# richardbaihe/a3t

Measured on AMD Instinct MI355X. Metric: mel-frames/sec (train), higher is better.
Workload: dtype bf16; 1 GPU; VCTK A3T masked-mel train step: 6+6 Conformer blocks d=384 H=2 ff=1536(k3), B=32/GPU, T_mel=1000, T_phn=120, postnet 5x256x5, fwd+bwd+clip+Adam, dropout 0.2/0.2/0.2 + postnet 0.5 (recipe); global_batch=32, parallelism=dp1, params=100799808

## Files before the change

a3t_amd/_lib.py:

```python
import ctypes
import os
from ctypes import POINTER, c_char_p, c_float, c_int, c_int32, c_int64, c_void_p

import torch

HERE = os.path.dirname(os.path.abspath(__file__))
LIB_PATH = os.environ.get("A3T_LIB_PATH") or os.path.join(HERE, "lib", "liba3t_hip.so")

F32, BF16 = 0, 1
ACT_NONE, ACT_RELU, ACT_TANH, ACT_SWISH = 0, 1, 2, 3
ACC_STORE, ACC_ADD, ACC_ATOMIC, ACC_SOLE = 0, 1, 2, 3


class GemmDesc(ctypes.Structure):
    _fields_ = [
        ("A", c_void_p), ("B", c_void_p), ("C", c_void_p), ("bias", c_void_p), ("R", c_void_p), ("S", c_void_p),
        ("M", c_int32), ("N", c_int32), ("K", c_int32),
        ("a_rs", c_int64), ("a_cs", c_int64),
        ("b_rs", c_int64), ("b_cs", c_int64), ("b_ts", c_int64),
        ("c_rs", c_int64),
        ("batch", c_int32), ("batch_inner", c_int32),
        ("a_bs0", c_int64), ("a_bs1", c_int64), ("b_bs0", c_int64), ("b_bs1", c_int64),
        ("c_bs0", c_int64), ("c_bs1", c_int64),
        ("taps", c_int32), ("pad", c_int32), ("dil", c_int32), ("Tseq", c_int32), ("kshift", c_int32),
        ("alpha", c_float),
        ("act", c_int32), ("accumulate", c_int32), ("splitk", c_int32),
        ("a_dtype", c_int32), ("b_dtype", c_int32), ("c_dtype", c_int32), ("compute", c_int32),
        ("s_dtype", c_int32), ("colsum_slots", c_int32),
        ("colsum", c_void_p), ("colsum_bs1", c_int64), ("colsum_scale", c_float), ("drop_key", ctypes.c_uint32),
        ("drop_p", c_float), ("colsum_ss", c_int32),
        ("keep_out", c_void_p), ("keep_in", c_void_p),
        ("a_signmask", c_int32), ("keep_layout", c_int32),
        ("A2", c_void_p), ("B2", c_void_p), ("b2_cs", c_int64), ("b2_bs0", c_int64), ("b2_bs1", c_int64), ("colsum2", c_void_p),
        ("a2_rs", c_int64), ("a_unaligned", c_int32),
    ]


_P = c_void_p
_SIGS = {
    "a3t_gemm": [POINTER(GemmDesc), _P],
    "a3t_gemm_plan": [POINTER(GemmDesc), c_char_p, c_int],
    "a3t_layernorm_fwd": [_P, _P, _P, _P, c_int, _P, _P, c_int, c_int, c_float, _P],
    "a3t_layernorm_bwd": [_P, c_int, _P, _P, _P, _P, _P, _P, _P, _P, _P, _P, c_float, c_int, c_int, c_float,
                          ctypes.c_uint32, _P],
    "a3t_col_reduce": [_P, c_int, _P, _P, _P, _P, c_int, c_int, c_int64, c_int, _P],
    "a3t_f64_to_f32_add": [_P, _P, c_int, c_float, _P],
    "a3t_bn_act_fwd": [_P, _P, _P, _P, _P, _P, _P, _P, _P, c_int, c_int, c_int, c_float, c_float, c_int, c_int, _P],
    "a3t_bn_act_bwd_a": [_P, c_int, _P, _P, _P, _P, _P, _P, c_int, c_int, c_int, _P],
    "a3t_bn_act_bwd_b": [_P, c_int, _P, _P, _P, _P, _P, _P, _P, _P, _P, c_int, c_int, c_int, c_int, _P],
    "a3t_glu_dwconv_fwd": [_P, c_int, _P, _P, _P, c_int, _P, c_int, c_int, c_int, c_int, _P],
    "a3t_glu_dwconv_bwd": [_P, _P, c_int, _P, c_int, _P, _P, c_int, _P, _P, _P, c_int, c_int, c_int, c_int, _P],
    "a3t_add_pos_bias": [_P, _P, _P, _P, _P, c_int, c_int, c_int, _P],
    "a3t_add_pos_bias_bwd": [_P, _P, _P, c_int, c_int, c_int, _P],
    "a3t_relpos_softmax_fwd": [_P, _P, c_int, _P, _P, c_int, c_int, c_int, c_int, c_int64, c_int64, c_int64, c_float, _P,
                               c_float, ctypes.c_uint32, _P],
    "a3t_relpos_softmax_bwd": [_P, c_int, _P, c_int, _P, _P, c_int, c_int, c_int, c_int, c_int64, c_int64, c_int64, c_float, _P,
                               c_float, c_int64, c_int64, ctypes.c_uint32, _P, _P],
    "a3t_attn_fwd_train": [_P, _P, _P, _P, _P, _P, _P, _P, _P, _P, _P, c_int, c_int, c_int, c_int, c_int64, c_int64, c_int64,
                           c_int64, c_float, c_float, ctypes.c_uint32, _P, _P, _P],
    "a3t_attn_scale_rows": [_P, _P, _P, c_int, c_int, c_int, c_int, _P],
    "a3t_attn_bwd_ds": [_P, _P, _P, _P, _P, _P, _P, c_int, c_int, c_int, c_int, c_int64, c_int64, c_int64, c_int64, c_float,
                        c_float, ctypes.c_uint32, c_int, c_int64, _P],
    "a3t_attn_fwd": [_P, _P, _P, _P, _P, _P, _P, _P, c_int, c_int, c_int, c_int, c_int64, c_int64, c_int64, c_int64,
                     c_float, c_float, ctypes.c_uint32, _P, _P, _P],
    "a3t_pwg_block": [_P, _P, _P, _P, _P, _P, _P, _P, c_int, c_int, c_int, _P],
    "a3t_mask_fill": [_P, _P, _P, _P, c_int, c_int, c_int, _P],
    "a3t_embed_finish_fwd": [_P, _P, _P, _P, _P, _P, _P, c_int, c_int, c_int, c_int, c_float, c_float, ctypes.c_uint32,
                             _P, _P],
    "a3t_embed_finish_bwd": [_P, _P, _P, _P, _P, _P, _P, _P, c_int, c_int, c_int, c_int, c_int, c_int, c_float, c_float,
                             ctypes.c_uint32, _P],
    "a3t_scale": [_P, _P, c_int64, c_float, _P],
    "a3t_axpy": [_P, _P, c_int64, c_float, _P],
    "a3t_attn_bias_fold": [_P, c_int32, c_int32, _P, _P, _P, _P],
    "a3t_scale_dev": [_P, _P, c_int64, _P, _P],
    "a3t_slice_rows": [_P, _P, c_int, c_int, c_int, c_int, c_int, c_int, _P],
    "a3t_cast_bf16": [_P, _P, c_int64, _P],
    "a3t_cast_bf16_conv_t": [_P, _P, _P, _P, c_int, c_int, c_int, c_int, _P],
    "a3t_split_bf16": [_P, _P, _P, c_int64, _P],
    "a3t_reflect_pad": [_P, _P, c_int, c_int, c_int, c_int, _P],
    "a3t_stft_amp": [_P, _P, c_int64, c_int, c_int, _P],
    "a3t_logmel_finish": [_P, _P, c_int, c_int, c_int, _P],
    "a3t_mlm_loss": [_P, _P, _P, _P, _P, _P, _P, _P, c_int, c_int, c_int, c_float, _P],
    "a3t_mlm_loss_scratch_floats": [c_int],
    "a3t_sumsq": [_P, c_int64, _P, _P],
# ... 62 lines not shown
```

a3t_amd/csrc/convmod_attn.hip:

```cpp
#include <hip/hip_runtime.h>
#include <stdint.h>
#include "../../include/a3t_hip.h"
#include "dtype_io.h"

#define WAVE 64
__device__ __forceinline__ float sigm(float v) { return 1.f / (1.f + __expf(-v)); }
__device__ __forceinline__ float bf2f_(unsigned int h) { return __uint_as_float(h << 16); }
__device__ __forceinline__ float wsum(float v) {
#pragma unroll
    for (int o = 32; o > 0; o >>= 1) v += __shfl_xor(v, o, WAVE);
    return v;
}
__device__ __forceinline__ float wmax(float v) {
#pragma unroll
    for (int o = 32; o > 0; o >>= 1) v = fmaxf(v, __shfl_xor(v, o, WAVE));
    return v;
}

#define DW_TT 64
#define DW_KMAX 31

template <int KT>
__global__ __launch_bounds__(256) void glu_dwconv_fwd_kernel(const void* __restrict__ g, int g_dt,
                                                             const float* __restrict__ wdw,
// ... 38 lines not shown
#pragma unroll
            for (int j = 0; j < KT + 3; ++j) v[j] = win[r0 + j][tx];
#pragma unroll
            for (int tt = 0; tt < 4; ++tt) {
                float acc = bias;
#pragma unroll
                for (int k = 0; k < KT; ++k) acc += w[k] * v[tt + k];
                int t = t0 + r0 + tt;
                if (t < Tseq) z[(mbase + t) * (int64_t)C + c] = acc;
            }
        }
        return;
    }
    for (int r = ty; r < DW_TT; r += 4) {
        int t = t0 + r;
        if (t >= Tseq) break;
        float acc = bias;
#pragma unroll
        for (int k = 0; k < KT; ++k)
            if (k < K) acc += w[k] * win[r + k][tx];
        z[(mbase + t) * (int64_t)C + c] = acc;
    }
}

int a3t_glu_dwconv_fwd_vec(const void* g, const float* wdw, const float* bdw, void* glu, float* z, int M, int C, int K,
                           int Tseq, hipStream_t stream);
int a3t_glu_dwconv_bwd_vec(const float* dz, const void* g, const void* glu, const float* wdw, void* dg, float* dwdw,
                           float* dbdw, float* dg_colsum, int M, int C, int K, int Tseq, hipStream_t stream);
static inline bool dw_al16(const void* p) { return ((uintptr_t)p & 15) == 0; }

extern "C" int a3t_glu_dwconv_fwd(const void* g, int g_dtype, const float* wdw, const float* bdw, void* glu,
                                  int glu_dtype, float* z, int M, int C, int K, int Tseq, void* stream) {
    if (K > DW_KMAX || (K & 1) == 0 || Tseq <= 0 || M % Tseq) return A3T_EINVAL;
    if (g_dtype == A3T_BF16 && glu_dtype == A3T_BF16 && C % 64 == 0 && dw_al16(g) && dw_al16(glu) && dw_al16(z))
        return a3t_glu_dwconv_fwd_vec(g, wdw, bdw, glu, z, M, C, K, Tseq, (hipStream_t)stream);
    int B = M / Tseq, tiles_t = (Tseq + DW_TT - 1) / DW_TT;
    dim3 grid((C + 63) / 64, B * tiles_t);
    if (K <= 7)
        hipLaunchKernelGGL(glu_dwconv_fwd_kernel<7>, grid, dim3(256), 0, (hipStream_t)stream, g, g_dtype, wdw, bdw, glu,
                           glu_dtype, z, C, K, Tseq, tiles_t);
    else if (K <= 15)
        hipLaunchKernelGGL(glu_dwconv_fwd_kernel<15>, grid, dim3(256), 0, (hipStream_t)stream, g, g_dtype, wdw, bdw, glu,
                           glu_dtype, z, C, K, Tseq, tiles_t);
    else
        hipLaunchKernelGGL(glu_dwconv_fwd_kernel<DW_KMAX>, grid, dim3(256), 0, (hipStream_t)stream, g, g_dtype, wdw, bdw,
                           glu, glu_dtype, z, C, K, Tseq, tiles_t);
    return (int)hipGetLastError();
}

template <int KT>
__global__ __launch_bounds__(256, 3) void glu_dwconv_bwd_kernel(const float* __restrict__ dz, const void* __restrict__ g,
                                                             int g_dt, const void* __restrict__ glu, int glu_dt,
                                                             const float* __restrict__ wdw, void* __restrict__ dg,
                                                             int dg_dt, float* dwdw, float* dbdw, float* dgsum, int C,
                                                             int K, int Tseq, int tiles_t, int tiles_per_block,
                                                             int chunks) {
    __shared__ float wdz[DW_TT + DW_KMAX - 1][64];
    __shared__ float wgl[DW_TT + DW_KMAX - 1][64];
    __shared__ float red[4][64];
    const int tx = threadIdx.x & 63, ty = threadIdx.x >> 6;
    const int c = blockIdx.x * 64 + tx;
    const int b = blockIdx.y / chunks, tile0 = (blockIdx.y % chunks) * tiles_per_block;
    const int pad = (K - 1) / 2;
    const int64_t mbase = (int64_t)b * Tseq;
    const int rows = DW_TT + K - 1;
    float w[KT], dw[KT];
#pragma unroll
    for (int k = 0; k < KT; ++k) {
// ... 661 lines not shown
```

a3t_amd/csrc/dwconv_vec.hip:

```cpp
#include <hip/hip_runtime.h>
#include <stdint.h>
#include "../../include/a3t_hip.h"
#include "dtype_io.h"

#define DW_TT 64
#define DW_KMAX 31
typedef unsigned short u16;

__device__ __forceinline__ float dv_sigm(float v) { return 1.f / (1.f + __expf(-v)); }
__device__ __forceinline__ float dv_bf(unsigned int h) { return __uint_as_float(h << 16); }
__device__ __forceinline__ void dv_unpack8(const uint4& u, float* f) {
    f[0] = dv_bf(u.x & 0xffff), f[1] = dv_bf(u.x >> 16), f[2] = dv_bf(u.y & 0xffff), f[3] = dv_bf(u.y >> 16);
    f[4] = dv_bf(u.z & 0xffff), f[5] = dv_bf(u.z >> 16), f[6] = dv_bf(u.w & 0xffff), f[7] = dv_bf(u.w >> 16);
}
__device__ __forceinline__ uint4 dv_pack8(const float* f) {
    uint4 u;
    u.x = io_pack2(f[0], f[1]), u.y = io_pack2(f[2], f[3]);
    u.z = io_pack2(f[4], f[5]), u.w = io_pack2(f[6], f[7]);
    return u;
}

template <int KT>
__global__ __launch_bounds__(256) void glu_dwconv_fwd_vec_kernel(const u16* __restrict__ g, const float* __restrict__ wdw,
                                                                 const float* __restrict__ bdw, u16* __restrict__ glu,
                                                                 float* __restrict__ z, int C, int K, int Tseq,
                                                                 int tiles_t) {
    __shared__ __attribute__((aligned(16))) float win[DW_TT + DW_KMAX - 1][64];
    __shared__ __attribute__((aligned(16))) float zt[DW_TT][64];
    const int tid = threadIdx.x, tx = tid & 63, ty = tid >> 6;
    const int cblk = blockIdx.x * 64, c = cblk + tx;
    const int b = blockIdx.y / tiles_t, t0 = (blockIdx.y % tiles_t) * DW_TT;
    const int pad = (K - 1) / 2;
    const int64_t mbase = (int64_t)b * Tseq;
    const int rows = DW_TT + K - 1;
    {
        const int rr = tid >> 3, c8 = (tid & 7) * 8;
        uint4 av[3], bv[3];
#pragma unroll
        for (int ps = 0; ps < 3; ++ps) {
            const int r = ps * 32 + rr, t = t0 - pad + r;
            const bool ok = (r < rows) && (t >= 0) && (t < Tseq);
            const u16* src = g + (ok ? (mbase + t) * (int64_t)(2 * C) + cblk + c8 : 0);
            av[ps] = *(const uint4*)src;
            bv[ps] = *(const uint4*)(src + (ok ? C : 0));
        }
#pragma unroll
        for (int ps = 0; ps < 3; ++ps) {
            const int r = ps * 32 + rr, t = t0 - pad + r;
            const bool ok = (r < rows) && (t >= 0) && (t < Tseq);
            if (r < rows) {
                float a[8], bb[8], v[8];
                dv_unpack8(av[ps], a);
                dv_unpack8(bv[ps], bb);
#pragma unroll
                for (int e = 0; e < 8; ++e) v[e] = ok ? a[e] * dv_sigm(bb[e]) : 0.f;
                *(float4*)&win[r][c8] = make_float4(v[0], v[1], v[2], v[3]);
                *(float4*)&win[r][c8 + 4] = make_float4(v[4], v[5], v[6], v[7]);
                if (ok && r >= pad && r < pad + DW_TT) *(uint4*)(glu + (mbase + t) * (int64_t)C + cblk + c8) = dv_pack8(v);
            }
        }
    }
    __syncthreads();
    float w[KT];
#pragma unroll
    for (int k = 0; k < KT; ++k) w[k] = (k < K) ? wdw[(int64_t)c * K + k] : 0.f;
    const float bias = bdw[c];
    if (K == KT) {
        for (int r0 = ty * 4; r0 < DW_TT; r0 += 16) {
            float v[KT + 3];
#pragma unroll
            for (int j = 0; j < KT + 3; ++j) v[j] = win[r0 + j][tx];
#pragma unroll
            for (int tt = 0; tt < 4; ++tt) {
                float acc = bias;
#pragma unroll
                for (int k = 0; k < KT; ++k) acc = __builtin_fmaf(w[k], v[tt + k], acc);
                zt[r0 + tt][tx] = acc;
            }
        }
    } else {
        for (int r = ty; r < DW_TT; r += 4) {
            float acc = bias;
#pragma unroll
            for (int k = 0; k < KT; ++k)
                if (k < K) acc += w[k] * win[r + k][tx];
            zt[r][tx] = acc;
        }
    }
    __syncthreads();
    {
        const int rr = tid >> 4, c4 = (tid & 15) * 4;
// ... 161 lines not shown
                if (t < Tseq) {
                    u16* dst = dg + (mbase + t) * (int64_t)(2 * C) + cblk + c8;
                    *(uint4*)dst = *(const uint4*)&gt[0][r][c8];
                    *(uint4*)(dst + C) = *(const uint4*)&gt[1][r][c8];
                }
            }
        }
    }
    __syncthreads();
    float* part = &wdz[0][0];
    for (int i = tid; i < 64 * K; i += 256) part[i] = 0.f;
    __syncthreads();
#pragma unroll
    for (int k = 0; k < KT; ++k)
        if (k < K) atomicAdd(&part[tx * K + k], dw[k]);
    __syncthreads();
    for (int i = tid; i < 64 * K; i += 256) atomicAdd(&dwdw[(int64_t)cblk * K + i], part[i]);
    __syncthreads();
    red[ty][tx] = db;
    __syncthreads();
    if (ty == 0) atomicAdd(&dbdw[c], red[0][tx] + red[1][tx] + red[2][tx] + red[3][tx]);
    if (dgsum) {
        __syncthreads();
        red[ty][tx] = sga;
        __syncthreads();
        if (ty == 0) atomicAdd(&dgsum[c], red[0][tx] + red[1][tx] + red[2][tx] + red[3][tx]);
        __syncthreads();
        red[ty][tx] = sgb;
        __syncthreads();
        if (ty == 0) atomicAdd(&dgsum[C + c], red[0][tx] + red[1][tx] + red[2][tx] + red[3][tx]);
    }
}

int a3t_glu_dwconv_bwd_vec(const float* dz, const void* g, const void* glu, const float* wdw, void* dg, float* dwdw,
                           float* dbdw, float* dg_colsum, int M, int C, int K, int Tseq, hipStream_t stream) {
    const int B = M / Tseq, tiles_t = (Tseq + DW_TT - 1) / DW_TT;
    const int cb = C / 64;
    int chunks = 1;
    while (cb * B * chunks < 640 && chunks < tiles_t) ++chunks;
    const int tpb = (tiles_t + chunks - 1) / chunks;
    chunks = (tiles_t + tpb - 1) / tpb;
    dim3 grid(cb, B * chunks);
#define DWB(KT)                                                                                                       \
    hipLaunchKernelGGL(glu_dwconv_bwd_vec_kernel<KT>, grid, dim3(256), 0, stream, dz, (const u16*)g, (const u16*)glu, \
                       wdw, (u16*)dg, dwdw, dbdw, dg_colsum, C, K, Tseq, tiles_t, tpb, chunks)
    if (K <= 7)
        DWB(7);
    else if (K <= 15)
        DWB(15);
    else
        DWB(DW_KMAX);
#undef DWB
    return (int)hipGetLastError();
}
```

a3t_amd/csrc/norm_reduce.hip:

```cpp
#include <hip/hip_runtime.h>
#include <stdlib.h>
#include <stdint.h>
#include "../../include/a3t_hip.h"
#include "dtype_io.h"

#define WAVE 64

__device__ __forceinline__ float wave_sum(float v) {
#pragma unroll
    for (int o = 32; o > 0; o >>= 1) v += __shfl_xor(v, o, WAVE);
    return v;
}

#define LN_MAXV 24

template <int V>
__global__ __launch_bounds__(256) void ln_fwd_kernel(const float* __restrict__ x, const float* __restrict__ g,
                                                     const float* __restrict__ b, void* __restrict__ y, int y_dt,
                                                     float* __restrict__ mean, float* __restrict__ rstd, int M,
                                                     int D, float eps) {
    const int lane = threadIdx.x & 63, wv = threadIdx.x >> 6;
    const int row = blockIdx.x * 4 + wv;
    if (row >= M) return;
    const float* xr = x + (int64_t)row * D;
    float v[V];
    float s = 0.f;
#pragma unroll
    for (int i = 0; i < V; ++i) {
        int c = lane + i * 64;
        v[i] = (c < D) ? xr[c] : 0.f;
        s += v[i];
    }
    const float mu = wave_sum(s) / (float)D;
    float q = 0.f;
#pragma unroll
    for (int i = 0; i < V; ++i) {
        int c = lane + i * 64;
// ... 382 lines not shown
}

__global__ void f64_to_f32_add_kernel(const double* src, float* dst, int n, float scale) {
    int i = blockIdx.x * blockDim.x + threadIdx.x;
    if (i < n) dst[i] += (float)(src[i] * (double)scale);
}
extern "C" int a3t_f64_to_f32_add(const double* src, float* dst, int n, float scale, void* stream) {
    hipLaunchKernelGGL(f64_to_f32_add_kernel, dim3((n + 255) / 256), dim3(256), 0, (hipStream_t)stream, src, dst, n,
                       scale);
    return (int)hipGetLastError();
}

__global__ void bn_finalize_kernel(const double* stats, float* running_mean, float* running_var, float* mean_out,
                                   float* rstd_out, int M, int C, float eps, float momentum, int training) {
    int c = blockIdx.x * blockDim.x + threadIdx.x;
    if (c >= C) return;
    if (training) {
        double mu = stats[c] / (double)M;
        double var = stats[C + c] / (double)M - mu * mu;
        if (var < 0.0) var = 0.0;
        mean_out[c] = (float)mu;
        rstd_out[c] = (float)(1.0 / sqrt(var + (double)eps));
        if (momentum > 0.f && running_mean) {
            double unb = (M > 1) ? var * (double)M / (double)(M - 1) : var;
            running_mean[c] = (1.f - momentum) * running_mean[c] + momentum * (float)mu;
            running_var[c] = (1.f - momentum) * running_var[c] + momentum * (float)unb;
        }
    } else {
        mean_out[c] = running_mean[c];
        rstd_out[c] = 1.0f / sqrtf(running_var[c] + eps);
    }
}

__device__ __forceinline__ float sigmoidf_(float v) { return 1.f / (1.f + __expf(-v)); }

__global__ __launch_bounds__(256) void bn_act_fwd_kernel(const float* __restrict__ z, const float* __restrict__ mean,
                                                         const float* __restrict__ rstd,
                                                         const float* __restrict__ gamma,
                                                         const float* __restrict__ beta, void* __restrict__ y,
                                                         int y_dt, int64_t n, int C, int act, int vec) {
    if (vec) {
        const int64_t n4 = n >> 2;
        for (int64_t q = (int64_t)blockIdx.x * blockDim.x + threadIdx.x; q < n4; q += (int64_t)gridDim.x * blockDim.x) {
            const int64_t i = q << 2;
            const int c = (int)(i % C);
            const float4 zv = *(const float4*)(z + i);
            const float4 mu = *(const float4*)(mean + c), rs = *(const float4*)(rstd + c);
            const float4 g = *(const float4*)(gamma + c), b = *(const float4*)(beta + c);
            float o[4] = {(zv.x - mu.x) * rs.x * g.x + b.x, (zv.y - mu.y) * rs.y * g.y + b.y,
                          (zv.z - mu.z) * rs.z * g.z + b.z, (zv.w - mu.w) * rs.w * g.w + b.w};
#pragma unroll
            for (int e = 0; e < 4; ++e) {
                if (act == A3T_ACT_SWISH)
                    o[e] = o[e] * sigmoidf_(o[e]);
                else if (act == A3T_ACT_TANH)
                    o[e] = tanhf(o[e]);
            }
            if (y_dt == A3T_BF16) {
                uint2 h;
                h.x = io_pack2(o[0], o[1]);
                h.y = io_pack2(o[2], o[3]);
                *(uint2*)((unsigned short*)y + i) = h;
            } else {
                *(float4*)((float*)y + i) = make_float4(o[0], o[1], o[2], o[3]);
            }
        }
        return;
    }
    for (int64_t i = (int64_t)blockIdx.x * blockDim.x + threadIdx.x; i < n; i += (int64_t)gridDim.x * blockDim.x) {
        int c = (int)(i % C);
        float bn = (z[i] - mean[c]) * rstd[c] * gamma[c] + beta[c];
        float o = bn;
        if (act == A3T_ACT_SWISH)
            o = bn * sigmoidf_(bn);
        else if (act == A3T_ACT_TANH)
            o = tanhf(bn);
        stx(y, y_dt, i, o);
    }
}

extern "C" int a3t_bn_act_fwd(const float* z, const double* stats, const float* gamma, const float* beta,
                              float* running_mean, float* running_var, float* mean_out, float* rstd_out, void* y,
                              int y_dtype, int M, int C, float eps, float momentum, int training, int act,
                              void* stream) {
    hipStream_t s = (hipStream_t)stream;
    hipLaunchKernelGGL(bn_finalize_kernel, dim3((C + 255) / 256), dim3(256), 0, s, stats, running_mean, running_var,
                       mean_out, rstd_out, M, C, eps, momentum, training);
    int64_t n = (int64_t)M * C;
    const int vec = (C % 4 == 0 && ((uintptr_t)z % 16 == 0) && ((uintptr_t)y % 16 == 0) && ((uintptr_t)mean_out % 16 == 0) &&
                     ((uintptr_t)rstd_out % 16 == 0) && ((uintptr_t)gamma % 16 == 0) && ((uintptr_t)beta % 16 == 0)) ? 1 : 0;
    int blocks = (int)(((vec ? n / 4 : n) + 255) / 256);
    if (blocks > 4096) blocks = 4096;
    hipLaunchKernelGGL(bn_act_fwd_kernel, dim3(blocks), dim3(256), 0, s, z, mean_out, rstd_out, gamma, beta, y, y_dtype, n,
                       C, act, vec);
    return (int)hipGetLastError();
}

__device__ __forceinline__ float bn_dact(float d, float bn, int act) {
    if (act == A3T_ACT_SWISH) {
        const float sg = sigmoidf_(bn);
        return d * sg * (1.f + bn * (1.f - sg));
    }
    if (act == A3T_ACT_TANH) {
        const float t = tanhf(bn);
        return d * (1.f - t * t);
    }
    return d;
}

__global__ __launch_bounds__(256) void bn_act_bwd_a_kernel(const void* __restrict__ dy, int dy_dt, const float* __restrict__ z,
                                                           const float* __restrict__ mean,
                                                           const float* __restrict__ rstd,
                                                           const float* __restrict__ gamma,
                                                           const float* __restrict__ beta,
                                                           double* sums, int M, int C, int act, int rows_per_block) {
    __shared__ double red[2][4][64];
    const int tx = threadIdx.x & 63, ty = threadIdx.x >> 6;
    const int c = blockIdx.x * 64 + tx;
    const int r0 = blockIdx.y * rows_per_block, r1 = min(M, r0 + rows_per_block);
    double a0 = 0.0, a1 = 0.0;
    if (c < C) {
        const float mu = mean[c], rs = rstd[c], g = gamma[c], b = beta[c];
        float f0 = 0.f, f1 = 0.f;
        int cnt = 0;
        for (int r = r0 + ty; r < r1; r += 4) {
            int64_t i = (int64_t)r * C + c;
            float zh = (z[i] - mu) * rs;
            float d = bn_dact(ldx(dy, dy_dt, i), zh * g + b, act);
            f0 += d;
            f1 += d * zh;
            if (++cnt == 32) {
                a0 += f0, a1 += f1, f0 = f1 = 0.f, cnt = 0;
            }
        }
        a0 += f0, a1 += f1;
    }
    red[0][ty][tx] = a0;
    red[1][ty][tx] = a1;
    __syncthreads();
    if (ty == 0 && c < C) {
// ... 118 lines not shown
```

a3t_amd/engine.py:

```python
import math
import os
import zlib
from typing import Dict

import torch

from . import ops
from ._lib import ACC_ADD, ACC_ATOMIC, ACC_STORE, ACT_NONE, ACT_RELU, ACT_SWISH, ACT_TANH, BF16, F32
from .config import A3TConfig
from .params import ParamStore


def legacy_pe_table(c: A3TConfig) -> torch.Tensor:
    d = c.adim
    position = torch.arange(c.max_len - 1, -1, -1.0, dtype=torch.float32).unsqueeze(1)
    div = torch.exp(torch.arange(0, d, 2, dtype=torch.float32) * -(math.log(10000.0) / d))
    pe = torch.zeros(c.max_len, d)
    pe[:, 0::2] = torch.sin(position * div)
    pe[:, 1::2] = torch.cos(position * div)
    return pe


_STREAMS = {}

# ... 653 lines not shown
            self._bias_grad(dqu, gr[pre + ".u"])
            self._bias_grad(dqv, gr[pre + ".v"])
            self._bias_grad(dqkv, gbq)
        self._lin_wgrad(dqkv, y, gr[pre + ".wqkv"])
        dy = self._act("tmp.dy", (M, d))
        self._lin_dgrad(dqkv, pre + ".wqkv", dy)
        self._pre_ln(ga, g, g16)
        self._ln_bwd(tag + ".ln", dy, pre + ".ln", g, g, g16, nb, nxt)
        self._sub_end()
        return g

    def _bn_fwd(self, tag, z, pre, bufpre, act, out):
        p, b = self.store.p, self.store.buf
        M, C = z.shape
        stats = self._arena_slot("fwd64", tag + ".stats", 2 * C)
        if self.training:
            ops.col_reduce(z, stats[:C], stats[C:], mode=1)
        mean = self.ws.get(tag + ".bnmean", (C,))
        rstd = self.ws.get(tag + ".bnrstd", (C,))
        ops.bn_act_fwd(z, stats, p[pre + ".g"], p[pre + ".b"], b[bufpre + ".rm"], b[bufpre + ".rv"], mean, rstd, out,
                       1e-5, self.bn_momentum if self.training else 0.0, self.training, act)
        if self.training:
            self.store.nbt[bufpre] = self.store.nbt.get(bufpre, 0) + 1
        self.sv[tag + ".bn"] = (z, mean, rstd)

    def _bn_bwd(self, tag, dy, pre, act, dz):
        p, gr = self.store.p, self.store.g
        z, mean, rstd = self.sv[tag + ".bn"]
        M, C = z.shape
        sums = self._arena_slot("bwd64", tag + ".bnsums", 2 * C)
        ops.bn_act_bwd(dy, z, mean, rstd, p[pre + ".g"], p[pre + ".b"], sums, dz, gr[pre + ".g"], gr[pre + ".b"],
                       self.training, act, zero=False)

    def _conv_fwd(self, tag, pre, x, T):
        p, c = self.store.p, self.c
        M, d = x.shape
        cmp = self.cmp
        y = self._ln_fwd(tag + ".ln", x, pre + ".ln")
        g2 = self._act(tag + ".g", (M, 2 * d))
        ops.linear_fwd(y, self.W(pre + ".pw1"), g2, bias=p[pre + ".pb1"], compute=cmp)
        glu = self._act(tag + ".glu", (M, d))
        z = self.ws.get(tag + ".z", (M, d))
        ops.glu_dwconv_fwd(g2, p[pre + ".dw"], p[pre + ".db"], glu, z, T)
        s = self._act(tag + ".s", (M, d))
        self._bn_fwd(tag, z, pre + ".bn", pre + ".bn", ACT_SWISH, s)
        xo = self.ws.get(tag + ".xo", (M, d))
        ops.linear_fwd(s, self.W(pre + ".pw2"), xo, bias=p[pre + ".pb2"], R=x, compute=cmp,
                       drop=self._drop(c.dropout_rate, tag + ".o"))
        self.sv[tag] = (y, g2, glu, s)
        return xo

    def _conv_bwd(self, tag, pre, g, T, nb=None, nxt=None):
        p, gr, c = self.store.p, self.store.g, self.c
        M, d = g.shape
        cmp = self.cmp
        y, g2, glu, s = self.sv[tag]
        self._sub_begin()
        g16 = self._g16(g)
        ga = self._gm(g, tag + ".o", c.dropout_rate, gr[pre + ".pb2"], 1.0)
        self._lin_wgrad(ga, s, gr[pre + ".pw2"])
        ds = self.ws.get("tmp.ds", (M, d))
        self._lin_dgrad(ga, pre + ".pw2", ds)
        dz = self.ws.get("tmp.dz", (M, d))
        self._bn_bwd(tag, ds, pre + ".bn", ACT_SWISH, dz)
        dg = self._act(self._t("tmp.dg"), (M, 2 * d))
        ops.glu_dwconv_bwd(dz, g2, glu, p[pre + ".dw"], dg, gr[pre + ".dw"], gr[pre + ".db"], T,
                           dgsum=gr[pre + ".pb1"])
        self._lin_wgrad(dg, y, gr[pre + ".pw1"])
        dy = self._act("tmp.dy", (M, d))
        self._lin_dgrad(dg, pre + ".pw1", dy)
        self._pre_ln(ga, g, g16)
        self._ln_bwd(tag + ".ln", dy, pre + ".ln", g, g, g16, nb, nxt)
        self._sub_end()
        return g

    def block_fwd(self, pre, x, pos, keymask, B, T):
        x = self._ffn_fwd(pre + ".ffm", pre + ".ffm", x, T)
        x = self._mha_fwd(pre + ".mha", pre + ".mha", x, pos, keymask, B, T)
        x = self._conv_fwd(pre + ".cnv", pre + ".cnv", x, T)
        x = self._ffn_fwd(pre + ".ff", pre + ".ff", x, T)
        return self._ln_fwd(pre + ".fin", x, pre + ".fin.ln", out_dtype=torch.float32)

    def block_bwd(self, pre, g, B, T):
        gr = self.store.g
        self._ln_bwd(pre + ".fin", g, pre + ".fin.ln", None, g, self._g16(g), (gr[pre + ".ff.b2"], 0.5), pre + ".ff.o")
        self._ffn_bwd(pre + ".ff", pre + ".ff", g, T, (gr[pre + ".cnv.pb2"], 1.0), pre + ".cnv.o")
        self._conv_bwd(pre + ".cnv", pre + ".cnv", g, T, (gr[pre + ".mha.bo"], 1.0), pre + ".mha.o")
        self._mha_bwd(pre + ".mha", pre + ".mha", g, B, T, (gr[pre + ".ffm.b2"], 0.5), pre + ".ffm.o")
        self._ffn_bwd(pre + ".ffm", pre + ".ffm", g, T, None)
        return g

    def forward(self, batch: Dict[str, torch.Tensor], need_grad: bool = True, gscale: float = 1.0):
        c, p, ws = self.c, self.store.p, self.ws
        speech = batch["speech"].contiguous()
        B, Tm, idim = speech.shape
        text = batch["text"].contiguous()
        Tp = text.shape[1]
        T = Tm + Tp
        d = c.adim
        if self.bf16 and (T % 8 or Tm % 8):
# ... 229 lines not shown
```

a3t_amd/ops.py:

```python
import ctypes
import os

import torch

from . import _lib as L
from ._lib import ACC_ADD, ACC_ATOMIC, ACC_SOLE, ACC_STORE, ACT_NONE, ACT_RELU, ACT_SWISH, ACT_TANH, BF16, F32

__all__ = ["gemm", "gemm_plan", "linear_fwd", "linear_bwd_data", "linear_bwd_weight", "conv_fwd", "conv_bwd_data",
           "conv_bwd_weight"]


PROFILE = None


def _stream():
    return ctypes.c_void_p(torch.cuda.current_stream().cuda_stream)


def _ptr(t):
    if t is None:
        return None
    return ctypes.c_void_p(t.data_ptr())


# ... 215 lines not shown

def layernorm_bwd(dy, x, g, mean, rstd, dres, dx, dg, db, dx16=None, dxsum=None, dxsum_scale=1.0, drop=(0.0, 0)):
    M, D = x.shape
    L.check(L.load().a3t_layernorm_bwd(_ptr(dy), _dt(dy), _ptr(x), _ptr(g), _ptr(mean), _ptr(rstd), _ptr(dres),
                                       _ptr(dx), _ptr(dx16), _ptr(dg), _ptr(db), _ptr(dxsum), dxsum_scale, M, D,
                                       drop[0], drop[1], _stream()), "ln_bwd")


def col_reduce(x, out0, out1=None, y=None, rowmask=None, mode=0, ld=None):
    M, C = x.shape
    L.check(L.load().a3t_col_reduce(_ptr(x), _dt(x), _ptr(y), _ptr(rowmask), _ptr(out0), _ptr(out1), M, C,
                                    ld if ld is not None else x.stride(0), mode, _stream()), "col_reduce")


def f64_to_f32_add(src, dst, scale=1.0):
    L.check(L.load().a3t_f64_to_f32_add(_ptr(src), _ptr(dst), dst.numel(), scale, _stream()), "f64_to_f32_add")


def bias_grad(dy, dbias, scratch64, scale=1.0):
    n = dy.shape[1]
    s = scratch64[:n]
    s.zero_()
    col_reduce(dy, s, mode=0)
    f64_to_f32_add(s, dbias, scale)


def bn_act_fwd(z, stats, g, b, rmean, rvar, mean_out, rstd_out, y, eps, momentum, training, act):
    M, C = z.shape
    L.check(L.load().a3t_bn_act_fwd(_ptr(z), _ptr(stats), _ptr(g), _ptr(b), _ptr(rmean), _ptr(rvar), _ptr(mean_out),
                                    _ptr(rstd_out), _ptr(y), _dt(y), M, C, eps, momentum, int(training), act,
                                    _stream()), "bn_act_fwd")


def bn_act_bwd(dy, z, mean, rstd, g, b, sums, dz, dg, db, training, act, zero=True):
    M, C = z.shape
    lib = L.load()
    if zero:
        sums.zero_()
    L.check(lib.a3t_bn_act_bwd_a(_ptr(dy), _dt(dy), _ptr(z), _ptr(mean), _ptr(rstd), _ptr(g), _ptr(b), _ptr(sums), M, C,
                                 act, _stream()), "bn_bwd_a")
    L.check(lib.a3t_bn_act_bwd_b(_ptr(dy), _dt(dy), _ptr(z), _ptr(mean), _ptr(rstd), _ptr(g), _ptr(b), _ptr(sums),
                                 _ptr(dz), _ptr(dg), _ptr(db), M, C, int(training), act, _stream()), "bn_bwd_b")


def glu_dwconv_fwd(g, wdw, bdw, glu, z, Tseq):
    M, C = glu.shape
    L.check(L.load().a3t_glu_dwconv_fwd(_ptr(g), _dt(g), _ptr(wdw), _ptr(bdw), _ptr(glu), _dt(glu), _ptr(z), M, C,
                                        wdw.shape[1], Tseq, _stream()), "glu_dwconv_fwd")


def glu_dwconv_bwd(dz, g, glu, wdw, dg, dwdw, dbdw, Tseq, dgsum=None):
    M, C = glu.shape
    L.check(L.load().a3t_glu_dwconv_bwd(_ptr(dz), _ptr(g), _dt(g), _ptr(glu), _dt(glu), _ptr(wdw), _ptr(dg), _dt(dg),
                                        _ptr(dwdw), _ptr(dbdw), _ptr(dgsum), M, C, wdw.shape[1], Tseq, _stream()),
            "glu_dwconv_bwd")


def add_pos_bias(qkv, u, v, qu, qv):
    M, d = qu.shape
    L.check(L.load().a3t_add_pos_bias(_ptr(qkv), _ptr(u), _ptr(v), _ptr(qu), _ptr(qv), _dt(qkv), M, d, _stream()),
            "pos_bias")


def add_pos_bias_bwd(dqu, dqv, dqkv):
    M, d = dqu.shape
    L.check(L.load().a3t_add_pos_bias_bwd(_ptr(dqu), _ptr(dqv), _ptr(dqkv), _dt(dqu), M, d, _stream()),
            "pos_bias_bwd")


def relpos_softmax_fwd(ac, bd, keymask, probs, B, H, T, scale, probs_drop=None, drop=(0.0, 0)):
    L.check(L.load().a3t_relpos_softmax_fwd(_ptr(ac), _ptr(bd), _dt(ac), _ptr(keymask), _ptr(probs), _dt(probs), B, H, T,
                                            T * T, T * T, T * T, scale, _ptr(probs_drop), drop[0], drop[1],
                                            _stream()), "softmax_fwd")


def relpos_softmax_bwd(probs, dprobs, ds, dbd, B, H, T, scale, probs_drop=None, drop_p=0.0, dbd_head_major=False,
                       drop_key=0, rowscale=None):
    bsb, bsh = (T * T, B * T * T) if dbd_head_major else (0, 0)
    L.check(L.load().a3t_relpos_softmax_bwd(_ptr(probs), _dt(probs), _ptr(dprobs), _dt(dprobs), _ptr(ds), _ptr(dbd), _dt(dbd), B, H,
                                            T, T * T, T * T, T * T, scale, _ptr(probs_drop), drop_p, bsb, bsh, drop_key,
                                            _ptr(rowscale), _stream()), "softmax_bwd")
# ... 198 lines not shown
```

include/a3t_hip.h:

```cpp
#ifndef A3T_HIP_H
#define A3T_HIP_H
#include <stdint.h>

#ifdef __cplusplus
extern "C" {
#endif

#define A3T_F32 0
#define A3T_BF16 1

#define A3T_EINVAL (-22)

#define A3T_ACT_NONE 0
#define A3T_ACT_RELU 1
#define A3T_ACT_TANH 2
#define A3T_ACT_SWISH 3

#define A3T_ACC_STORE 0
#define A3T_ACC_ADD 1
#define A3T_ACC_ATOMIC 2
#define A3T_ACC_SOLE 3

typedef struct a3t_gemm_desc {
    const void* A;
// ... 37 lines not shown

int a3t_gemm(const a3t_gemm_desc* d, void* stream);
int a3t_gemm_plan(const a3t_gemm_desc* d, char* name, int len);
int a3t_gemm_8p_supported(int M, int N, int K, int taps, int flags);
int64_t a3t_gemm_keep_bytes(int M, int N);
int a3t_gemm_pn_supported(int M, int N, int K, int taps, int flags);
int a3t_gemm_tt_supported(int M, int N, int K, int batch);

int a3t_layernorm_fwd(const float* x, const float* gamma, const float* beta, void* y, int y_dtype,
                      float* mean, float* rstd, int M, int D, float eps, void* stream);
int a3t_layernorm_bwd(const void* dy, int dy_dtype, const float* x, const float* gamma, const float* mean,
                      const float* rstd, const float* dres, float* dx, void* dx_bf16, float* dgamma,
                      float* dbeta, float* dx_colsum, float dx_colsum_scale, int M, int D, float drop_p,
                      uint32_t drop_key, void* stream);

int a3t_col_reduce(const void* x, int x_dtype, const float* y, const uint8_t* rowmask, double* out0,
                   double* out1, int M, int C, int64_t ld, int mode, void* stream);
int a3t_f64_to_f32_add(const double* src, float* dst, int n, float scale, void* stream);

int a3t_bn_act_fwd(const float* z, const double* stats, const float* gamma, const float* beta,
                   float* running_mean, float* running_var, float* mean_out, float* rstd_out, void* y,
                   int y_dtype, int M, int C, float eps, float momentum, int training, int act, void* stream);
int a3t_bn_act_bwd_a(const void* dy, int dy_dtype, const float* z, const float* mean, const float* rstd,
                     const float* gamma, const float* beta, double* sums, int M, int C, int act, void* stream);
int a3t_bn_act_bwd_b(const void* dy, int dy_dtype, const float* z, const float* mean, const float* rstd,
                     const float* gamma, const float* beta, const double* sums, float* dz, float* dgamma,
                     float* dbeta, int M, int C, int training, int act, void* stream);

int a3t_glu_dwconv_fwd(const void* g, int g_dtype, const float* wdw, const float* bdw, void* glu,
                       int glu_dtype, float* z, int M, int C, int K, int Tseq, void* stream);
int a3t_glu_dwconv_bwd(const float* dz, const void* g, int g_dtype, const void* glu, int glu_dtype,
                       const float* wdw, void* dg, int dg_dtype, float* dwdw, float* dbdw, float* dg_colsum,
                       int M, int C, int K, int Tseq, void* stream);

int a3t_add_pos_bias(const void* qkv, const float* bias_u, const float* bias_v, void* qu, void* qv, int dtype,
                     int M, int d, void* stream);
int a3t_add_pos_bias_bwd(const void* dqu, const void* dqv, void* dqkv, int dtype, int M, int d, void* stream);
int a3t_relpos_softmax_fwd(const void* ac, const void* bd, int scores_dtype, const uint8_t* keymask, void* probs,
                           int probs_dtype, int B, int H, int T, int64_t ac_bs, int64_t bd_bs, int64_t p_bs,
                           float scale, void* probs_drop, float drop_p, uint32_t drop_key, void* stream);
int a3t_relpos_softmax_bwd(const void* probs, int probs_dtype, const void* dprobs, int dprobs_dtype, void* ds,
                           void* dbd, int out_dtype, int B, int H, int T, int64_t p_bs, int64_t dp_bs, int64_t o_bs,
                           float scale, const void* probs_drop, float drop_p, int64_t dbd_bs_b, int64_t dbd_bs_h,
                           uint32_t drop_key, const float* rowscale, void* stream);

int a3t_attn_fwd(const void* qu, const void* qv, const void* k, const void* v, const void* pos, const uint8_t* keymask,
                 void* ctx, float* lse, int B, int H, int T, int dk, int64_t ldq, int64_t ldkv, int64_t ldp, int64_t ldo,
                 float scale, float drop_p, uint32_t drop_key, const float* bias_u, const float* bias_v, void* stream);

int a3t_attn_fwd_train(const void* qu, const void* qv, const void* k, const void* v, const void* pos,
                       const uint8_t* keymask, void* ctx, float* lse, void* probs, void* probs_drop, float* rowscale,
                       int B, int H, int T, int dk, int64_t ldq, int64_t ldkv, int64_t ldp, int64_t ldo, float scale,
                       float drop_p, uint32_t drop_key, const float* bias_u, const float* bias_v, void* stream);
int a3t_attn_scale_rows(const void* x, const float* rowscale, void* y, int B, int H, int T, int dk, void* stream);
int a3t_attn_bwd_ds(const void* dctx, const void* ctx, const void* v, const void* probs, const float* rowscale, void* ds,
                    void* dbd, int B, int H, int T, int dk, int64_t ldo, int64_t ldkv, int64_t dbd_bsb, int64_t dbd_bsh,
                    float scale, float drop_p, uint32_t drop_key, int signed_probs, int64_t ds_bs, void* stream);

int a3t_mask_fill(const float* speech, const uint8_t* masked, const float* mask_feature, void* out,
                  int out_dtype, int M, int C, void* stream);
int a3t_embed_finish_fwd(const float* e, const float* emb, const float* seg, const int64_t* text,
                         const int64_t* spos, const int64_t* tpos, float* xs, int B, int Tm, int Tp, int D,
                         float xscale, float drop_p, uint32_t drop_key, const float* spk, void* stream);
int a3t_embed_finish_bwd(const float* dxs, const float* e, const int64_t* text, const int64_t* spos,
                         const int64_t* tpos, float* de, float* demb, float* dseg, int B, int Tm, int Tp,
                         int D, int V, int nseg, float xscale, float drop_p, uint32_t drop_key, void* stream);
// ... 68 lines not shown
```

Measured before the change: 801,400 mel-frames/s.

## Fuse BN-swish backward into GLU depthwise-conv backward and drop saved GLU

Result: no change. 808,500 mel-frames/s (median of 6 runs) (+0.9%).

```diff
diff --git a/a3t_amd/_lib.py b/a3t_amd/_lib.py
--- a/a3t_amd/_lib.py
+++ b/a3t_amd/_lib.py
@@ -50,6 +50,8 @@
     "a3t_bn_act_bwd_b": [_P, c_int, _P, _P, _P, _P, _P, _P, _P, _P, _P, c_int, c_int, c_int, c_int, _P],
     "a3t_glu_dwconv_fwd": [_P, c_int, _P, _P, _P, c_int, _P, c_int, c_int, c_int, c_int, _P],
     "a3t_glu_dwconv_bwd": [_P, _P, c_int, _P, c_int, _P, _P, c_int, _P, _P, _P, c_int, c_int, c_int, c_int, _P],
+    "a3t_bnswish_glu_dwconv_bwd": [_P, _P, _P, _P, _P, _P, _P, _P, _P, _P, _P, _P, _P, _P, _P, c_int, c_int, c_int, c_int,
+                                   c_int, _P],
     "a3t_add_pos_bias": [_P, _P, _P, _P, _P, c_int, c_int, c_int, _P],
     "a3t_add_pos_bias_bwd": [_P, _P, _P, c_int, c_int, c_int, _P],
     "a3t_relpos_softmax_fwd": [_P, _P, c_int, _P, _P, c_int, c_int, c_int, c_int, c_int64, c_int64, c_int64, c_float, _P,
diff --git a/a3t_amd/csrc/bn_act.h b/a3t_amd/csrc/bn_act.h
--- /dev/null
+++ b/a3t_amd/csrc/bn_act.h
@@ -0,0 +1,17 @@
+#pragma once
+#include <hip/hip_runtime.h>
+#include "../../include/a3t_hip.h"
+
+__device__ __forceinline__ float sigmoidf_(float v) { return 1.f / (1.f + __expf(-v)); }
+
+__device__ __forceinline__ float bn_dact(float d, float bn, int act) {
+    if (act == A3T_ACT_SWISH) {
+        const float sg = sigmoidf_(bn);
+        return d * sg * (1.f + bn * (1.f - sg));
+    }
+    if (act == A3T_ACT_TANH) {
+        const float t = tanhf(bn);
+        return d * (1.f - t * t);
+    }
+    return d;
+}
diff --git a/a3t_amd/csrc/convmod_attn.hip b/a3t_amd/csrc/convmod_attn.hip
--- a/a3t_amd/csrc/convmod_attn.hip
+++ b/a3t_amd/csrc/convmod_attn.hip
@@ -94,8 +94,9 @@
 extern "C" int a3t_glu_dwconv_fwd(const void* g, int g_dtype, const float* wdw, const float* bdw, void* glu,
                                   int glu_dtype, float* z, int M, int C, int K, int Tseq, void* stream) {
     if (K > DW_KMAX || (K & 1) == 0 || Tseq <= 0 || M % Tseq) return A3T_EINVAL;
-    if (g_dtype == A3T_BF16 && glu_dtype == A3T_BF16 && C % 64 == 0 && dw_al16(g) && dw_al16(glu) && dw_al16(z))
+    if (g_dtype == A3T_BF16 && (glu_dtype == A3T_BF16 || !glu) && C % 64 == 0 && dw_al16(g) && dw_al16(glu) && dw_al16(z))
         return a3t_glu_dwconv_fwd_vec(g, wdw, bdw, glu, z, M, C, K, Tseq, (hipStream_t)stream);
+    if (!glu) return A3T_EINVAL;
     int B = M / Tseq, tiles_t = (Tseq + DW_TT - 1) / DW_TT;
     dim3 grid((C + 63) / 64, B * tiles_t);
     if (K <= 7)
diff --git a/a3t_amd/csrc/dwconv_vec.hip b/a3t_amd/csrc/dwconv_vec.hip
--- a/a3t_amd/csrc/dwconv_vec.hip
+++ b/a3t_amd/csrc/dwconv_vec.hip
@@ -2,6 +2,7 @@
 #include <stdint.h>
 #include "../../include/a3t_hip.h"
 #include "dtype_io.h"
+#include "bn_act.h"
 
 #define DW_TT 64
 #define DW_KMAX 31
@@ -56,7 +57,8 @@
                 for (int e = 0; e < 8; ++e) v[e] = ok ? a[e] * dv_sigm(bb[e]) : 0.f;
                 *(float4*)&win[r][c8] = make_float4(v[0], v[1], v[2], v[3]);
                 *(float4*)&win[r][c8 + 4] = make_float4(v[4], v[5], v[6], v[7]);
-                if (ok && r >= pad && r < pad + DW_TT) *(uint4*)(glu + (mbase + t) * (int64_t)C + cblk + c8) = dv_pack8(v);
+                if (glu && ok && r >= pad && r < pad + DW_TT)
+                    *(uint4*)(glu + (mbase + t) * (int64_t)C + cblk + c8) = dv_pack8(v);
             }
         }
     }
@@ -284,15 +286,21 @@
     }
 }
 
+static dim3 dw_bwd_grid(int M, int C, int Tseq, int* tiles_t, int* tpb, int* chunks) {
+    const int B = M / Tseq;
+    *tiles_t = (Tseq + DW_TT - 1) / DW_TT;
+    const int cb = C / 64;
+    int ch = 1;
+    while (cb * B * ch < 640 && ch < *tiles_t) ++ch;
+    *tpb = (*tiles_t + ch - 1) / ch;
+    *chunks = (*tiles_t + *tpb - 1) / *tpb;
+    return dim3(cb, B * *chunks);
+}
+
 int a3t_glu_dwconv_bwd_vec(const float* dz, const void* g, const void* glu, const float* wdw, void* dg, float* dwdw,
                            float* dbdw, float* dg_colsum, int M, int C, int K, int Tseq, hipStream_t stream) {
-    const int B = M / Tseq, tiles_t = (Tseq + DW_TT - 1) / DW_TT;
-    const int cb = C / 64;
-    int chunks = 1;
-    while (cb * B * chunks < 640 && chunks < tiles_t) ++chunks;
-    const int tpb = (tiles_t + chunks - 1) / chunks;
-    chunks = (tiles_t + tpb - 1) / tpb;
-    dim3 grid(cb, B * chunks);
+    int tiles_t, tpb, chunks;
+    const dim3 grid = dw_bwd_grid(M, C, Tseq, &tiles_t, &tpb, &chunks);
 #define DWB(KT)                                                                                                       \
     hipLaunchKernelGGL(glu_dwconv_bwd_vec_kernel<KT>, grid, dim3(256), 0, stream, dz, (const u16*)g, (const u16*)glu, \
                        wdw, (u16*)dg, dwdw, dbdw, dg_colsum, C, K, Tseq, tiles_t, tpb, chunks)
@@ -305,3 +313,223 @@
 #undef DWB
     return (int)hipGetLastError();
 }
+
+__device__ __forceinline__ float4 dv_bnswish_dz(const float4& s, const float4& zv, const float (*bnc)[64], int c4,
+                                                int training) {
+    const float dd[4] = {s.x, s.y, s.z, s.w}, zz[4] = {zv.x, zv.y, zv.z, zv.w};
+    float o[4];
+#pragma unroll
+    for (int e = 0; e < 4; ++e) {
+        const float mm = bnc[0][c4 + e], rr = bnc[1][c4 + e], gg = bnc[2][c4 + e], bb = bnc[3][c4 + e];
+        const float zh = (zz[e] - mm) * rr;
+        float d = bn_dact(dd[e], zh * gg + bb, A3T_ACT_SWISH);
+        if (training) d = d - bnc[4][c4 + e] - zh * bnc[5][c4 + e];
+        o[e] = gg * rr * d;
+    }
+    return make_float4(o[0], o[1], o[2], o[3]);
+}
+
+template <int KT>
+__global__ __launch_bounds__(256, 3) void bnswish_glu_dwconv_bwd_vec_kernel(
+    const float* __restrict__ ds, const float* __restrict__ z, const float* __restrict__ mean,
+    const float* __restrict__ rstd, const float* __restrict__ gamma, const float* __restrict__ beta,
+    const double* __restrict__ sums, const u16* __restrict__ g, const float* __restrict__ wdw, u16* __restrict__ dg,
+    float* dwdw, float* dbdw, float* dgsum, float* dgamma, float* dbeta, int M, int C, int K, int Tseq, int tiles_t,
+    int tiles_per_block, int chunks, int training) {
+    __shared__ __attribute__((aligned(16))) float wdz[DW_TT + DW_KMAX - 1 + 6][64];
+    __shared__ __attribute__((aligned(16))) u16 gt[2][DW_TT][64];
+    __shared__ float red[4][64];
+    float (*bnc)[64] = &wdz[DW_TT + DW_KMAX - 1];
+    const int tid = threadIdx.x, tx = tid & 63, ty = tid >> 6;
+    const int cblk = blockIdx.x * 64, c = cblk + tx;
+    const int b = blockIdx.y / chunks, tile0 = (blockIdx.y % chunks) * tiles_per_block;
+    const int pad = (K - 1) / 2, halo = 2 * pad;
+    const int64_t mbase = (int64_t)b * Tseq;
+    if (ty == 0) {
+        const double invM = 1.0 / (double)M;
+        bnc[0][tx] = mean[c], bnc[1][tx] = rstd[c], bnc[2][tx] = gamma[c], bnc[3][tx] = beta[c];
+        bnc[4][tx] = (float)(sums[c] * invM), bnc[5][tx] = (float)(sums[C + c] * invM);
+    }
+    float w[KT], dw[KT];
+#pragma unroll
+    for (int k = 0; k < KT; ++k) {
+        w[k] = (k < K) ? wdw[(int64_t)c * K + k] : 0.f;
+        dw[k] = 0.f;
+    }
+    float db = 0.f, sga = 0.f, sgb = 0.f;
+    const int r16 = tid >> 4, c4 = (tid & 15) * 4;
+    const int r32 = tid >> 3, c8 = (tid & 7) * 8;
+    __syncthreads();
+    {
+        const int t0 = tile0 * DW_TT;
+        for (int r = r16; r < halo; r += 16) {
+            const int t = t0 - pad + r;
+            float4 v = make_float4(0.f, 0.f, 0.f, 0.f);
+            if (t >= 0 && t < Tseq) {
+                const int64_t off = (mbase + t) * (int64_t)C + cblk + c4;
+                v = dv_bnswish_dz(*(const float4*)(ds + off), *(const float4*)(z + off), bnc, c4, training);
+            }
+            *(float4*)&wdz[r][c4] = v;
+        }
+    }
+    for (int tile = tile0; tile < min(tiles_t, tile0 + tiles_per_block); ++tile) {
+        const int t0 = tile * DW_TT;
+        __syncthreads();
+        {
+            float4 vs[4], vz[4];
+            uint4 va[2], vb[2];
+#pragma unroll
+            for (int ps = 0; ps < 4; ++ps) {
+                const int t = t0 + pad + ps * 16 + r16;
+                vs[ps] = vz[ps] = make_float4(0.f, 0.f, 0.f, 0.f);
+                if (t < Tseq) {
+                    vs[ps] = *(const float4*)(ds + (mbase + t) * (int64_t)C + cblk + c4);
+                    vz[ps] = *(const float4*)(z + (mbase + t) * (int64_t)C + cblk + c4);
+                }
+            }
+#pragma unroll
+            for (int ps = 0; ps < 2; ++ps) {
+                const int r = ps * 32 + r32, t = t0 + r;
+                const bool ok = t < Tseq;
+                const u16* src = g + (ok ? (mbase + t) * (int64_t)(2 * C) + cblk + c8 : 0);
+                va[ps] = *(const uint4*)src;
+                vb[ps] = *(const uint4*)(src + (ok ? C : 0));
+            }
+#pragma unroll
+            for (int ps = 0; ps < 4; ++ps) {
+                const int t = t0 + pad + ps * 16 + r16;
+                *(float4*)&wdz[halo + ps * 16 + r16][c4] =
+                    t < Tseq ? dv_bnswish_dz(vs[ps], vz[ps], bnc, c4, training) : make_float4(0.f, 0.f, 0.f, 0.f);
+            }
+#pragma unroll
+            for (int ps = 0; ps < 2; ++ps) {
+                const int r = ps * 32 + r32;
+                *(uint4*)&gt[0][r][c8] = va[ps];
+                *(uint4*)&gt[1][r][c8] = vb[ps];
+            }
+        }
+        __syncthreads();
+        if (K == KT) {
+#pragma unroll 1
+            for (int i = 0; i < 4; ++i) {
+                const int r0 = ty * 4 + 16 * i;
+                float u[KT + 3], ga[4], sb[4], gl[4], acc[4];
+#pragma unroll
+                for (int j = 0; j < KT + 3; ++j) u[j] = wdz[r0 + j][tx];
+#pragma unroll
+                for (int tt = 0; tt < 4; ++tt) {
+                    const int r = r0 + tt;
+                    ga[tt] = dv_bf(gt[0][r][tx]), sb[tt] = dv_sigm(dv_bf(gt[1][r][tx]));
+                    gl[tt] = (t0 + r < Tseq) ? dv_bf(io_f2bf(ga[tt] * sb[tt])) : 0.f;
+                }
+#pragma unroll
+                for (int tt = 0; tt < 4; ++tt) {
+                    float a = 0.f;
+#pragma unroll
+                    for (int k = 0; k < KT; ++k) {
+                        const float v = u[tt + KT - 1 - k];
+                        a = __builtin_fmaf(w[k], v, a);
+                        dw[k] = __builtin_fmaf(gl[tt], v, dw[k]);
+                    }
+                    acc[tt] = a;
+                    db += u[tt + (KT - 1) / 2];
+                }
+#pragma unroll
+                for (int tt = 0; tt < 4; ++tt) {
+                    const int r = r0 + tt;
+                    const float da = acc[tt] * sb[tt], dbb = acc[tt] * ga[tt] * sb[tt] * (1.f - sb[tt]);
+                    gt[0][r][tx] = io_f2bf(da);
+                    gt[1][r][tx] = io_f2bf(dbb);
+                    if (t0 + r < Tseq) sga += da, sgb += dbb;
+                }
+            }
+        } else {
+            for (int r = ty; r < DW_TT; r += 4) {
+                const float ga = dv_bf(gt[0][r][tx]), sb = dv_sigm(dv_bf(gt[1][r][tx]));
+                const float gl = (t0 + r < Tseq) ? dv_bf(io_f2bf(ga * sb)) : 0.f;
+                float acc = 0.f;
+#pragma unroll
+                for (int k = 0; k < KT; ++k)
+                    if (k < K) {
+                        const float v = wdz[r + 2 * pad - k][tx];
+                        acc += w[k] * v;
+                        dw[k] += gl * v;
+                    }
+                const float da = acc * sb, dbb = acc * ga * sb * (1.f - sb);
+                gt[0][r][tx] = io_f2bf(da);
+                gt[1][r][tx] = io_f2bf(dbb);
+                if (t0 + r < Tseq) sga += da, sgb += dbb;
+                db += wdz[r + pad][tx];
+            }
+        }
+        __syncthreads();
+        {
+            const int r32 = tid >> 3, c8 = (tid & 7) * 8;
+#pragma unroll
+            for (int ps = 0; ps < 2; ++ps) {
+                const int r = ps * 32 + r32, t = t0 + r;
+                if (t < Tseq) {
+                    u16* dst = dg + (mbase + t) * (int64_t)(2 * C) + cblk + c8;
+                    *(uint4*)dst = *(const uint4*)&gt[0][r][c8];
+                    *(uint4*)(dst + C) = *(const uint4*)&gt[1][r][c8];
+                }
+            }
+        }
+        for (int i = tid; i < halo * 16; i += 256) {
+            const int r = i >> 4, q = (i & 15) * 4;
+            *(float4*)&wdz[r][q] = *(const float4*)&wdz[r + DW_TT][q];
+        }
+    }
+    __syncthreads();
+    float* part = &wdz[0][0];
+    for (int i = tid; i < 64 * K; i += 256) part[i] = 0.f;
+    __syncthreads();
+#pragma unroll
+    for (int k = 0; k < KT; ++k)
+        if (k < K) atomicAdd(&part[tx * K + k], dw[k]);
+    __syncthreads();
+    for (int i = tid; i < 64 * K; i += 256) atomicAdd(&dwdw[(int64_t)cblk * K + i], part[i]);
+    __syncthreads();
+    red[ty][tx] = db;
+    __syncthreads();
+    if (ty == 0) {
+        atomicAdd(&dbdw[c], red[0][tx] + red[1][tx] + red[2][tx] + red[3][tx]);
+        if (blockIdx.y == 0) {
+            dgamma[c] += (float)sums[C + c];
+            dbeta[c] += (float)sums[c];
+        }
+    }
+    if (dgsum) {
+        __syncthreads();
+        red[ty][tx] = sga;
+        __syncthreads();
+        if (ty == 0) atomicAdd(&dgsum[c], red[0][tx] + red[1][tx] + red[2][tx] + red[3][tx]);
+        __syncthreads();
+        red[ty][tx] = sgb;
+        __syncthreads();
+        if (ty == 0) atomicAdd(&dgsum[C + c], red[0][tx] + red[1][tx] + red[2][tx] + red[3][tx]);
+    }
+}
+
+extern "C" int a3t_bnswish_glu_dwconv_bwd(const float* ds, const float* z, const float* mean, const float* rstd,
+                                          const float* gamma, const float* beta, const double* sums, const void* g,
+                                          const float* wdw, void* dg, float* dwdw, float* dbdw, float* dg_colsum,
+                                          float* dgamma, float* dbeta, int M, int C, int K, int Tseq, int training,
+                                          void* stream) {
+    if (K > DW_KMAX || (K & 1) == 0 || Tseq <= 0 || M <= 0 || M % Tseq || C <= 0 || C % 64) return A3T_EINVAL;
+    if (((uintptr_t)ds | (uintptr_t)z | (uintptr_t)g | (uintptr_t)dg) & 15) return A3T_EINVAL;
+    int tiles_t, tpb, chunks;
+    const dim3 grid = dw_bwd_grid(M, C, Tseq, &tiles_t, &tpb, &chunks);
+#define DWF(KT)                                                                                                          \
+    hipLaunchKernelGGL(bnswish_glu_dwconv_bwd_vec_kernel<KT>, grid, dim3(256), 0, (hipStream_t)stream, ds, z, mean, rstd, \
+                       gamma, beta, sums, (const u16*)g, wdw, (u16*)dg, dwdw, dbdw, dg_colsum, dgamma, dbeta, M, C, K,   \
+                       Tseq, tiles_t, tpb, chunks, training)
+    if (K <= 7)
+        DWF(7);
+    else if (K <= 15)
+        DWF(15);
+    else
+        DWF(DW_KMAX);
+#undef DWF
+    return (int)hipGetLastError();
+}
diff --git a/a3t_amd/csrc/norm_reduce.hip b/a3t_amd/csrc/norm_reduce.hip
--- a/a3t_amd/csrc/norm_reduce.hip
+++ b/a3t_amd/csrc/norm_reduce.hip
@@ -3,6 +3,7 @@
 #include <stdint.h>
 #include "../../include/a3t_hip.h"
 #include "dtype_io.h"
+#include "bn_act.h"
 
 #define WAVE 64
 
@@ -451,8 +452,6 @@
     }
 }
 
-__device__ __forceinline__ float sigmoidf_(float v) { return 1.f / (1.f + __expf(-v)); }
-
 __global__ __launch_bounds__(256) void bn_act_fwd_kernel(const float* __restrict__ z, const float* __restrict__ mean,
                                                          const float* __restrict__ rstd,
                                                          const float* __restrict__ gamma,
@@ -513,18 +512,6 @@
     hipLaunchKernelGGL(bn_act_fwd_kernel, dim3(blocks), dim3(256), 0, s, z, mean_out, rstd_out, gamma, beta, y, y_dtype, n,
                        C, act, vec);
     return (int)hipGetLastError();
-}
-
-__device__ __forceinline__ float bn_dact(float d, float bn, int act) {
-    if (act == A3T_ACT_SWISH) {
-        const float sg = sigmoidf_(bn);
-        return d * sg * (1.f + bn * (1.f - sg));
-    }
-    if (act == A3T_ACT_TANH) {
-        const float t = tanhf(bn);
-        return d * (1.f - t * t);
-    }
-    return d;
 }
 
 __global__ __launch_bounds__(256) void bn_act_bwd_a_kernel(const void* __restrict__ dy, int dy_dt, const float* __restrict__ z,
diff --git a/a3t_amd/engine.py b/a3t_amd/engine.py
--- a/a3t_amd/engine.py
+++ b/a3t_amd/engine.py
@@ -709,6 +709,9 @@
         ops.bn_act_bwd(dy, z, mean, rstd, p[pre + ".g"], p[pre + ".b"], sums, dz, gr[pre + ".g"], gr[pre + ".b"],
                        self.training, act, zero=False)
 
+    def _conv_fused(self, d):
+        return self.bf16 and d % 64 == 0
+
     def _conv_fwd(self, tag, pre, x, T):
         p, c = self.store.p, self.c
         M, d = x.shape
@@ -716,7 +719,7 @@
         y = self._ln_fwd(tag + ".ln", x, pre + ".ln")
         g2 = self._act(tag + ".g", (M, 2 * d))
         ops.linear_fwd(y, self.W(pre + ".pw1"), g2, bias=p[pre + ".pb1"], compute=cmp)
-        glu = self._act(tag + ".glu", (M, d))
+        glu = None if self._conv_fused(d) else self._act(tag + ".glu", (M, d))
         z = self.ws.get(tag + ".z", (M, d))
         ops.glu_dwconv_fwd(g2, p[pre + ".dw"], p[pre + ".db"], glu, z, T)
         s = self._act(tag + ".s", (M, d))
@@ -738,11 +741,20 @@
         self._lin_wgrad(ga, s, gr[pre + ".pw2"])
         ds = self.ws.get("tmp.ds", (M, d))
         self._lin_dgrad(ga, pre + ".pw2", ds)
-        dz = self.ws.get("tmp.dz", (M, d))
-        self._bn_bwd(tag, ds, pre + ".bn", ACT_SWISH, dz)
         dg = self._act(self._t("tmp.dg"), (M, 2 * d))
-        ops.glu_dwconv_bwd(dz, g2, glu, p[pre + ".dw"], dg, gr[pre + ".dw"], gr[pre + ".db"], T,
-                           dgsum=gr[pre + ".pb1"])
+        if glu is None:
+            z, mean, rstd = self.sv[tag + ".bn"]
+            sums = self._arena_slot("bwd64", tag + ".bnsums", 2 * d)
+            bn = pre + ".bn"
+            ops.bn_act_bwd_sums(ds, z, mean, rstd, p[bn + ".g"], p[bn + ".b"], sums, ACT_SWISH)
+            ops.bnswish_glu_dwconv_bwd(ds, z, mean, rstd, p[bn + ".g"], p[bn + ".b"], sums, g2, p[pre + ".dw"], dg,
+                                       gr[pre + ".dw"], gr[pre + ".db"], gr[bn + ".g"], gr[bn + ".b"], T, self.training,
+                                       dgsum=gr[pre + ".pb1"])
+        else:
+            dz = self.ws.get("tmp.dz", (M, d))
+            self._bn_bwd(tag, ds, pre + ".bn", ACT_SWISH, dz)
+            ops.glu_dwconv_bwd(dz, g2, glu, p[pre + ".dw"], dg, gr[pre + ".dw"], gr[pre + ".db"], T,
+                               dgsum=gr[pre + ".pb1"])
         self._lin_wgrad(dg, y, gr[pre + ".pw1"])
         dy = self._act("tmp.dy", (M, d))
         self._lin_dgrad(dg, pre + ".pw1", dy)
diff --git a/a3t_amd/ops.py b/a3t_amd/ops.py
--- a/a3t_amd/ops.py
+++ b/a3t_amd/ops.py
@@ -271,21 +271,35 @@
                                     _stream()), "bn_act_fwd")
 
 
+def bn_act_bwd_sums(dy, z, mean, rstd, g, b, sums, act):
+    M, C = z.shape
+    L.check(L.load().a3t_bn_act_bwd_a(_ptr(dy), _dt(dy), _ptr(z), _ptr(mean), _ptr(rstd), _ptr(g), _ptr(b), _ptr(sums),
+                                      M, C, act, _stream()), "bn_bwd_a")
+
+
 def bn_act_bwd(dy, z, mean, rstd, g, b, sums, dz, dg, db, training, act, zero=True):
     M, C = z.shape
     lib = L.load()
     if zero:
         sums.zero_()
-    L.check(lib.a3t_bn_act_bwd_a(_ptr(dy), _dt(dy), _ptr(z), _ptr(mean), _ptr(rstd), _ptr(g), _ptr(b), _ptr(sums), M, C,
-                                 act, _stream()), "bn_bwd_a")
+    bn_act_bwd_sums(dy, z, mean, rstd, g, b, sums, act)
     L.check(lib.a3t_bn_act_bwd_b(_ptr(dy), _dt(dy), _ptr(z), _ptr(mean), _ptr(rstd), _ptr(g), _ptr(b), _ptr(sums),
                                  _ptr(dz), _ptr(dg), _ptr(db), M, C, int(training), act, _stream()), "bn_bwd_b")
 
 
 def glu_dwconv_fwd(g, wdw, bdw, glu, z, Tseq):
-    M, C = glu.shape
-    L.check(L.load().a3t_glu_dwconv_fwd(_ptr(g), _dt(g), _ptr(wdw), _ptr(bdw), _ptr(glu), _dt(glu), _ptr(z), M, C,
-                                        wdw.shape[1], Tseq, _stream()), "glu_dwconv_fwd")
+    M, C = z.shape
+    L.check(L.load().a3t_glu_dwconv_fwd(_ptr(g), _dt(g), _ptr(wdw), _ptr(bdw), _ptr(glu), _dt(glu) if glu is not None else BF16,
+                                        _ptr(z), M, C, wdw.shape[1], Tseq, _stream()), "glu_dwconv_fwd")
+
+
+def bnswish_glu_dwconv_bwd(ds, z, mean, rstd, gamma, beta, sums, g, wdw, dg, dwdw, dbdw, dgamma, dbeta, Tseq, training,
+                           dgsum=None):
+    M, C = z.shape
+    L.check(L.load().a3t_bnswish_glu_dwconv_bwd(_ptr(ds), _ptr(z), _ptr(mean), _ptr(rstd), _ptr(gamma), _ptr(beta),
+                                                _ptr(sums), _ptr(g), _ptr(wdw), _ptr(dg), _ptr(dwdw), _ptr(dbdw),
+                                                _ptr(dgsum), _ptr(dgamma), _ptr(dbeta), M, C, wdw.shape[1], Tseq,
+                                                int(training), _stream()), "bnswish_glu_dwconv_bwd")
 
 
 def glu_dwconv_bwd(dz, g, glu, wdw, dg, dwdw, dbdw, Tseq, dgsum=None):
diff --git a/include/a3t_hip.h b/include/a3t_hip.h
--- a/include/a3t_hip.h
+++ b/include/a3t_hip.h
@@ -93,6 +93,10 @@
 int a3t_glu_dwconv_bwd(const float* dz, const void* g, int g_dtype, const void* glu, int glu_dtype,
                        const float* wdw, void* dg, int dg_dtype, float* dwdw, float* dbdw, float* dg_colsum,
                        int M, int C, int K, int Tseq, void* stream);
+int a3t_bnswish_glu_dwconv_bwd(const float* ds, const float* z, const float* mean, const float* rstd,
+                               const float* gamma, const float* beta, const double* sums, const void* g,
+                               const float* wdw, void* dg, float* dwdw, float* dbdw, float* dg_colsum, float* dgamma,
+                               float* dbeta, int M, int C, int K, int Tseq, int training, void* stream);
 
 int a3t_add_pos_bias(const void* qkv, const float* bias_u, const float* bias_v, void* qu, void* qv, int dtype,
                      int M, int d, void* stream);
```
